# zju3dv/pvnet

Measured on NVIDIA H100. Metric: images/sec (480x640, K=9) backbone+vote, higher is better.
Workload: dtype tf32 (fp32 storage, fp32 accumulate; vote fp32/fp64)

## Files before the change

pvnet_b200/csrc/conv_col.cu:

```cuda
#include "conv_tc.cuh"
#include "ptx.cuh"

#include <cstdlib>
#include <mutex>
#include <new>

namespace pvnet {

int g_conv_mode = 0;

namespace {

constexpr int COL_TH = 16, COL_TW = 8;
constexpr int COL_THREADS = 384;
constexpr int HEAD_MAX = 64;

__host__ __device__ constexpr int head_pitch(int hc) { return hc <= 8 ? 8 : (hc <= 24 ? 24 : 40); }
constexpr int HEAD_CPITCH = COL_TH * COL_TW + 4;
__host__ __device__ constexpr int head_stage_floats(int hc)
{
    return COL_TH * COL_TW * head_pitch(hc) > hc * HEAD_CPITCH ? COL_TH * COL_TW * head_pitch(hc) : hc * HEAD_CPITCH;
}
__host__ __device__ constexpr int head_stage_bytes(int hc) { return (head_stage_floats(hc) * 4 + COL_TH * COL_TW + 127) & ~127; }

struct ColGeom {
    int Ho, Wo, tiles_x, tiles_y, total_tiles;
    int cin_chunks, cin_pad;
    int split_chunk;
    int pad_l, pad_t;
    int stages;
    int resident;
    int out_cs, out_co, res_cs, res_co;
    int act, round_out;
    int head_cout, head_seg, mask_esz;
    int head_nhwc;
};

__device__ __forceinline__ void head_store_tile(const ColGeom &g, uint32_t sv, uint32_t sm, float *head_out, void *mask,
                                                int img, int y0, int x0, int tid, int nthr)
{
    const int hc = g.head_cout, pp = head_pitch(hc);
    const int nx = min(COL_TW, g.Wo - x0), ny = min(COL_TH, g.Ho - y0);
    const size_t npix = (size_t)g.Ho * g.Wo;
    const bool vec = (reinterpret_cast<uintptr_t>(head_out) & 15) == 0 && (g.head_nhwc ? hc % 4 == 0 : g.Wo % 4 == 0);
    for (int u = tid; u < 32 * hc; u += nthr) {
        if (g.head_nhwc) {
            const int r = u / (2 * hc), e0 = 4 * (u - r * 2 * hc);
            if (r >= ny) continue;
            float *dst = head_out + (((size_t)img * g.Ho + y0 + r) * g.Wo + x0) * hc + e0;
            if (vec) {
                const int col = e0 / hc;
                if (col < nx)
                    *reinterpret_cast<float4 *>(dst) = ptx::lds128(sv + 4u * (uint32_t)((r * COL_TW + col) * pp + e0 - col * hc));
            } else {
#pragma unroll
                for (int i = 0; i < 4; ++i) {
                    const int col = (e0 + i) / hc;
                    if (col < nx) dst[i] = ptx::lds32(sv + 4u * (uint32_t)((r * COL_TW + col) * pp + e0 + i - col * hc));
                }
            }
        } else {
            const int co = u >> 5, r = (u >> 1) & 15, xo = 4 * (u & 1);
            if (r >= ny) continue;
            float *dst = head_out + ((size_t)img * hc + co) * npix + (size_t)(y0 + r) * g.Wo + x0 + xo;
            const uint32_t src = sv + 4u * (uint32_t)(co * HEAD_CPITCH + r * COL_TW + xo);
            if (vec) {
                if (xo < nx) *reinterpret_cast<float4 *>(dst) = ptx::lds128(src);
            } else {
#pragma unroll
                for (int i = 0; i < 4; ++i)
                    if (xo + i < nx) dst[i] = ptx::lds32(src + 4u * i);
            }
        }
    }
    if (!mask) return;
    for (int p = tid; p < COL_TH * COL_TW; p += nthr) {
        const int r = p / COL_TW, c = p % COL_TW;
        if (r >= ny || c >= nx) continue;
        const size_t pix = ((size_t)img * g.Ho + y0 + r) * g.Wo + x0 + c;
        const uint32_t v = ptx::lds8(sm + (uint32_t)p);
        if (g.mask_esz == 8) reinterpret_cast<long long *>(mask)[pix] = v;
        else reinterpret_cast<unsigned char *>(mask)[pix] = (unsigned char)v;
    }
}

template <int KC, bool HEAD, int KH, int BN, bool WIDE = false>
__global__ void __launch_bounds__(COL_THREADS, 1)
    k_conv_col(const __grid_constant__ CUtensorMap tmA, const __grid_constant__ CUtensorMap tmA2,
               const __grid_constant__ CUtensorMap tmB, const __grid_constant__ CUtensorMap tmBw, const __grid_constant__ ColGeom g,
               const float *__restrict__ bias, const float *__restrict__ res, float *__restrict__ out,
               const float *__restrict__ head_w, const float *__restrict__ head_b, float *__restrict__ head_out,
               void *__restrict__ mask)
{
    static_assert(!HEAD || BN == 32, "fused head: 32 input channels");
    static_assert(!HEAD || KC == 8, "fused head: convraw.0's 8-channel chunks");
    static_assert((KC == 16) == (KH == 4), "16-channel chunks are the 4x4 stem's, and only its");
    static_assert(!WIDE || (HEAD && KC == 8 && KH == 3), "wide first source: convraw.0 form only");
    constexpr int ROWB = KC * 4;
    constexpr int B_TILE = BN * ROWB;
    constexpr int PITCH = COL_TW + KH - 1;
    constexpr int A_BOX = (COL_TH + KH - 1) * PITCH * ROWB;
    constexpr int A_BYTES = (A_BOX + 1023) & ~1023;
    constexpr int WIDE_BOX = (COL_TH + KH - 1) * PITCH * 128;
    constexpr int WIDE_BYTES = (WIDE_BOX + 1023) & ~1023;
    extern __shared__ uint8_t smem_raw[];
    uint8_t *smem = reinterpret_cast<uint8_t *>((reinterpret_cast<uintptr_t>(smem_raw) + 1023) & ~uintptr_t(1023));
    const int n_btiles = KH * KH * g.cin_chunks;
    const int n_loads = WIDE ? 2 : g.cin_chunks;
    const int stage_bytes = WIDE ? WIDE_BYTES : A_BYTES + (g.resident ? 0 : KH * KH * B_TILE);
    uint8_t *sB = smem;
    uint8_t *sA = smem + (g.resident ? (size_t)n_btiles * B_TILE : 0);
    uint8_t *sH = sA + (size_t)g.stages * stage_bytes;
    uint8_t *sHS = sH + (HEAD ? 4096 : 0);
    const int hs_bytes = HEAD ? head_stage_bytes(g.head_cout) : 0;
    uint64_t *wfull = reinterpret_cast<uint64_t *>(sHS + 2 * hs_bytes);
    uint64_t *full = wfull + 1;
    uint64_t *empty = full + g.stages;
    uint64_t *hstaged = empty + g.stages;
    uint64_t *hfree = hstaged + 2;
    float *s_bias = reinterpret_cast<float *>(empty + g.stages + (HEAD ? 4 : 0));
    float *s_head = s_bias + 64;
    constexpr int STORE_THREADS = 96;

    const int warp = threadIdx.x >> 5, lane = threadIdx.x & 31;
    if (threadIdx.x == 0) {
        ptx::mbar_init(wfull, 1);
        for (int s = 0; s < g.stages; ++s) {
            ptx::mbar_init(&full[s], 1);
            ptx::mbar_init(&empty[s], 8);
        }
        if (HEAD)
            for (int b = 0; b < 2; ++b) {
                ptx::mbar_init(&hstaged[b], 256);
                ptx::mbar_init(&hfree[b], STORE_THREADS);
            }
        ptx::fence_barrier_init();
    }
    for (int i = threadIdx.x; i < BN; i += blockDim.x) s_bias[i] = bias[i];
    if (HEAD) {
        for (int i = threadIdx.x; i < 32; i += blockDim.x) s_head[i] = i < g.head_cout ? head_b[i] : 0.f;
        for (int i = threadIdx.x; i < 32 * 32; i += blockDim.x) {
            const int n = i >> 5, p = i & 31, q = p & 7;
            const int k = (p & ~7) + (q < 4 ? 2 * q : 2 * (q - 4) + 1);
            const float v = n < g.head_cout ? head_w[n * 32 + k] : 0.f;
            *reinterpret_cast<float *>(sH + ptx::swizzle_off((uint32_t)(n * 128 + p * 4), 128)) = v;
        }
        ptx::fence_proxy_async();
    }
    __syncthreads();
    const int tiles_per_img = g.tiles_x * g.tiles_y;

    if (warp >= 8) {
        const int pw = warp - 8;
        if (pw == 0 && lane == 0 && g.resident) {
            ptx::mbar_arrive_expect_tx(wfull, (uint32_t)(n_btiles * B_TILE));
            for (int cc = WIDE ? g.split_chunk : 0; cc < g.cin_chunks; ++cc)
                for (int t = 0; t < KH * KH; ++t)
                    ptx::tma_load_2d(sB + (size_t)(cc * KH * KH + t) * B_TILE, &tmB, wfull, t * g.cin_pad + cc * KC, 0);
            if (WIDE)
                for (int t = 0; t < KH * KH; ++t) ptx::tma_load_2d(sB + (size_t)t * BN * 128, &tmBw, wfull, t * g.cin_pad, 0);
        }
        if (HEAD && pw != 0) {
            const int tid = threadIdx.x - 9 * 32;
            int it = 0;
            for (int tile = blockIdx.x; tile < g.total_tiles; tile += gridDim.x, ++it) {
                const int b = it & 1;
                const int img = tile / tiles_per_img;
                const int trem = tile - img * tiles_per_img;
                const int tyi = trem / g.tiles_x, txi = trem - tyi * g.tiles_x;
                const uint32_t buf = ptx::smem_u32(sHS) + (uint32_t)(b * hs_bytes);
                ptx::mbar_wait(&hstaged[b], (uint32_t)(it >> 1) & 1u);
                head_store_tile(g, buf, buf + 4u * (uint32_t)head_stage_floats(g.head_cout), head_out, mask, img, tyi * COL_TH,
                                txi * COL_TW, tid, STORE_THREADS);
                ptx::mbar_arrive(&hfree[b]);
            }
            return;
        }
        if (pw != 0) return;
        int s = 0;
        uint32_t ph = 0;
        const uint32_t tx_bytes = (uint32_t)(A_BOX + (g.resident ? 0 : KH * KH * B_TILE));
        for (int tile = blockIdx.x; tile < g.total_tiles; tile += gridDim.x) {
            const int img = tile / tiles_per_img;
            const int trem = tile - img * tiles_per_img;
            const int tyi = trem / g.tiles_x, txi = trem - tyi * g.tiles_x;
            const int y0 = tyi * COL_TH, x0 = txi * COL_TW;
            for (int cc = 0; cc < n_loads; ++cc) {
                uint8_t *st = sA + (size_t)s * stage_bytes;
                if (WIDE) {
                    if (pw == 0 && lane == 0) {
                        ptx::mbar_wait(&empty[s], ph ^ 1u);
                        ptx::mbar_arrive_expect_tx(&full[s], (uint32_t)(cc == 0 ? WIDE_BOX : A_BOX));
                        ptx::tma_load_4d(st, cc == 0 ? &tmA : &tmA2, &full[s], 0, x0 - g.pad_l, y0 - g.pad_t, img);
                    }
                    __syncwarp();
                } else if (pw == 0) {
                    if (lane == 0) {
                        ptx::mbar_wait(&empty[s], ph ^ 1u);
                        ptx::mbar_arrive_expect_tx(&full[s], tx_bytes);
                        if (cc < g.split_chunk)
                            ptx::tma_load_4d(st, &tmA, &full[s], cc * KC, x0 - g.pad_l, y0 - g.pad_t, img);
                        else
                            ptx::tma_load_4d(st, &tmA2, &full[s], (cc - g.split_chunk) * KC, x0 - g.pad_l, y0 - g.pad_t, img);
                        if (!g.resident)
                            for (int t = 0; t < KH * KH; ++t)
                                ptx::tma_load_2d(st + A_BYTES + (size_t)t * B_TILE, &tmB, &full[s], t * g.cin_pad + cc * KC, 0);
                    }
                    __syncwarp();
                }
                if (++s == g.stages) {
                    s = 0;
                    ph ^= 1u;
                }
            }
        }
        return;
    }

    const int wg = warp >> 2, wq = warp & 3;
    const int g8 = lane >> 2, t4 = lane & 3;
    const uint32_t sA_u = ptx::smem_u32(sA), sB_u = ptx::smem_u32(sB);
    if (g.resident) ptx::mbar_wait(wfull, 0);
    int s = 0;
    uint32_t ph = 0;
    int it = 0;
    for (int tile = blockIdx.x; tile < g.total_tiles; tile += gridDim.x, ++it) {
        float acc[BN / 2];
#pragma unroll
        for (int i = 0; i < BN / 2; ++i) acc[i] = 0.f;
        int prev = -1;
        for (int cc = 0; cc < n_loads; ++cc) {
            ptx::mbar_wait(&full[s], ph);
            const uint32_t a0 = sA_u + (uint32_t)s * (uint32_t)stage_bytes;
            ptx::wgmma_fence();
            if (WIDE && cc == 0) {
                const uint64_t ad0 = ptx::make_kmajor_desc(a0 + (uint32_t)(8 * wg * PITCH * 128), 128, PITCH * 128);
                const uint64_t bd0 = ptx::make_kmajor_desc(sB_u, 128);
#pragma unroll
                for (int ks = 0; ks < 4; ++ks)
#pragma unroll
                    for (int t = 0; t < KH * KH; ++t)
                        ptx::Wgmma<BN>::ss(acc, ad0 + (uint64_t)(((t / KH) * PITCH + t % KH) * 128 / 16 + 2 * ks),
                                           bd0 + (uint64_t)(t * (BN * 128) / 16 + 2 * ks), (t | ks) != 0 ? 1u : 0u);
            } else {
                const int c8 = WIDE ? g.split_chunk : cc;
                const uint32_t b0 = g.resident ? sB_u + (uint32_t)(c8 * KH * KH * B_TILE) : a0 + (uint32_t)A_BYTES;
                const uint64_t ad0 = ptx::make_kmajor_desc(a0 + (uint32_t)(8 * wg * PITCH * ROWB), ROWB, PITCH * ROWB);
                const uint64_t bd0 = ptx::make_kmajor_desc(b0, ROWB);
#pragma unroll
                for (int t = 0; t < KH * KH; ++t) {
                    const uint64_t ad = ad0 + (uint64_t)(((t / KH) * PITCH + t % KH) * ROWB / 16);
                    const uint64_t bd = bd0 + (uint64_t)(t * B_TILE / 16);
#pragma unroll
                    for (int ks = 0; ks < KC / 8; ++ks)
                        ptx::Wgmma<BN>::ss(acc, ad + (uint64_t)(2 * ks), bd + (uint64_t)(2 * ks), (c8 | t | ks) != 0 ? 1u : 0u);
                }
            }
            ptx::wgmma_commit();
            ptx::wgmma_wait<1>();
            ptx::fence_regs(acc);
            if (prev >= 0 && lane == 0) ptx::mbar_arrive(&empty[prev]);
            prev = s;
            if (++s == g.stages) {
                s = 0;
                ph ^= 1u;
            }
        }
        ptx::wgmma_wait<0>();
        ptx::fence_regs(acc);
        if (lane == 0) ptx::mbar_arrive(&empty[prev]);

        const int img = tile / tiles_per_img;
        const int trem = tile - img * tiles_per_img;
        const int tyi = trem / g.tiles_x, txi = trem - tyi * g.tiles_x;
        const int ty = 8 * wg + 2 * wq;
        if constexpr (!HEAD) {
            bool ok[2];
            size_t pix[2];
#pragma unroll
            for (int h = 0; h < 2; ++h) {
                const int y = tyi * COL_TH + ty + h, x = txi * COL_TW + g8;
                ok[h] = y < g.Ho && x < g.Wo;
                pix[h] = ok[h] ? ((size_t)img * g.Ho + y) * g.Wo + x : 0;
            }
            float2 rv[2][BN / 8];
            if (res) {
#pragma unroll
                for (int h = 0; h < 2; ++h)
#pragma unroll
                    for (int j = 0; j < BN / 8; ++j)
                        rv[h][j] = ok[h] ? __ldg(reinterpret_cast<const float2 *>(res + pix[h] * g.res_cs + g.res_co + 8 * j + 2 * t4))
                                         : make_float2(0.f, 0.f);
            }
#pragma unroll
            for (int h = 0; h < 2; ++h) {
                if (!ok[h]) continue;
                float *optr = out + pix[h] * g.out_cs + g.out_co;
#pragma unroll
                for (int j = 0; j < BN / 8; ++j) {
                    const int c = 8 * j + 2 * t4;
                    float2 v = make_float2(acc[4 * j + 2 * h] + s_bias[c], acc[4 * j + 2 * h + 1] + s_bias[c + 1]);
                    if (res) {
                        v.x += rv[h][j].x;
                        v.y += rv[h][j].y;
                    }
                    v.x = epi_act(v.x, g.act, g.round_out);
                    v.y = epi_act(v.y, g.act, g.round_out);
                    *reinterpret_cast<float2 *>(optr + c) = v;
                }
            }
        } else {
            uint32_t a2[4][4];
#pragma unroll
            for (int j = 0; j < 4; ++j)
#pragma unroll
                for (int f = 0; f < 4; ++f) {
                    const int r = 4 * j + ((f & 1) << 1) + (f >> 1);
                    const int c = 8 * j + 2 * t4 + (f >> 1);
                    a2[j][f] = __float_as_uint(ptx::round_tf32(epi_act(acc[r] + s_bias[c], g.act, g.round_out)));
                }
            float hacc[16];
#pragma unroll
            for (int i = 0; i < 16; ++i) hacc[i] = 0.f;
            const uint64_t hd = ptx::make_kmajor_desc(ptx::smem_u32(sH), 128);
            ptx::wgmma_fence();
#pragma unroll
            for (int j = 0; j < 4; ++j) ptx::Wgmma<32>::rs(hacc, a2[j], hd + (uint64_t)(2 * j), j != 0 ? 1u : 0u);
            ptx::wgmma_commit();
            ptx::wgmma_wait<0>();
            ptx::fence_regs(hacc);
            const int hc = g.head_cout, pp = head_pitch(hc);
            const uint32_t sv = ptx::smem_u32(sHS) + (uint32_t)((it & 1) * hs_bytes);
            const uint32_t sm = sv + 4u * (uint32_t)head_stage_floats(hc);
            ptx::mbar_wait(&hfree[it & 1], ((uint32_t)(it >> 1) & 1u) ^ 1u);
#pragma unroll
            for (int h = 0; h < 2; ++h) {
                const uint32_t p = (uint32_t)((ty + h) * COL_TW + g8);
                float best = -INFINITY;
                int best_c = 0;
#pragma unroll
                for (int j = 0; j < 4; ++j) {
                    const int co = 8 * j + 2 * t4;
                    float val[2];
#pragma unroll
                    for (int e = 0; e < 2; ++e) {
                        val[e] = hacc[4 * j + 2 * h + e] + s_head[co + e];
                        if (co + e < g.head_seg && val[e] > best) {
                            best = val[e];
                            best_c = co + e;
                        }
                    }
                    if (co < hc) {
                        if (g.head_nhwc) {
                            ptx::sts64(sv + 4u * (p * pp + co), make_float2(val[0], val[1]));
                        } else {
                            ptx::sts32(sv + 4u * (co * HEAD_CPITCH + p), val[0]);
                            if (co + 1 < hc) ptx::sts32(sv + 4u * ((co + 1) * HEAD_CPITCH + p), val[1]);
                        }
                    }
                }
#pragma unroll
                for (int o = 1; o < 4; o <<= 1) {
                    const float ob = __shfl_xor_sync(0xffffffffu, best, o);
                    const int oc = __shfl_xor_sync(0xffffffffu, best_c, o);
                    if (ob > best || (ob == best && oc < best_c)) {
                        best = ob;
                        best_c = oc;
                    }
                }
                if (t4 == 0) ptx::sts8(sm + p, (uint32_t)best_c);
            }
            ptx::mbar_arrive(&hstaged[it & 1]);
        }
    }
}

struct ColPlan {
    CUtensorMap tmA, tmA2, tmB, tmBw;
    ColGeom g;
    int kc, ksize, head, bn, wide;
    unsigned grid;
    size_t smem;
    const float *bias, *res;
    float *out;
    HeadDesc hd;
};

constexpr size_t SMEM_LIMIT = 227 * 1024;

int col_kc(int Cin) { return Cin % 32 == 0 ? 32 : (Cin == 16 ? 16 : 8); }
int col_cin_pad(int Cin) { return Cin == 16 ? 16 : (Cin + 31) / 32 * 32; }

size_t col_smem(int kc, int ksize, int cin_chunks, int bn, int stages, bool head, bool resident)
{
    const size_t rowb = (size_t)kc * 4;
    const size_t a_box = (size_t)(COL_TH + ksize - 1) * (COL_TW + ksize - 1) * rowb;
    const size_t a = (a_box + 1023) & ~(size_t)1023, bt = (size_t)bn * rowb;
    return 1024 + (resident ? (size_t)ksize * ksize * cin_chunks * bt : 0) +
           (size_t)stages * (a + (resident ? 0 : (size_t)ksize * ksize * bt)) + (head ? 4096 : 0) +
           (size_t)(1 + 2 * stages) * 8 + (64 + 32) * 4;
}

template <int KC, bool HEAD, int KH, int BN, bool WIDE = false>
int col_launch(const ColPlan &p, cudaStream_t s)
{
    if (p.bn != BN || p.kc != KC || p.ksize != KH || p.head != (HEAD ? 1 : 0) || p.wide != (WIDE ? 1 : 0)) {
        set_error("conv(col): no kernel instantiation for this plan (Cout %d, chunk %d, ksize %d)", p.bn, p.kc, p.ksize);
        return PVNET_E_STATE;
    }
    auto fn = k_conv_col<KC, HEAD, KH, BN, WIDE>;
    const cudaError_t attr_err = ensure_max_smem((const void *)fn, (int)SMEM_LIMIT);
    PV_CUDA(attr_err);
    const HeadDesc &h = p.hd;
    fn<<<p.grid, COL_THREADS, p.smem, s>>>(p.tmA, p.tmA2, p.tmB, p.tmBw, p.g, p.bias, p.res, p.out, p.head ? h.w : nullptr,
                                           p.head ? h.bias : nullptr, p.head ? h.out_nchw : nullptr,
                                           p.head ? h.mask : nullptr);
    PV_LAUNCHED("k_conv_col");
    return PVNET_OK;
}

}

bool conv_col_eligible(const ConvDesc &d)
{
    if ((d.ksize != 3 && d.ksize != 4) || d.stride != 1 || d.dilation != 1 || d.Cout > 64 || d.Cout % 32 != 0)
        return false;
    const int cin = d.Cin + d.Cin2;
    const int kc = col_kc(cin);
    if (d.Cin % kc != 0 || d.Cin2 % kc != 0) return false;
    if ((d.ksize == 4) != (kc == 16)) return false;
    return col_smem(kc, d.ksize, (cin + kc - 1) / kc, d.Cout, 2, true, false) <= SMEM_LIMIT;
}

size_t conv_col_plan_size() { return sizeof(ColPlan); }

int conv_col_plan_at(const ConvDesc &d, const HeadDesc *head, void *storage)
{
    ColPlan *p = new (storage) ColPlan();
    PV_CHECK_ARG(conv_col_eligible(d), "conv(col): layer not eligible for the column kernel");
    PV_CHECK_ARG(d.in && d.w && d.bias && (d.out || head), "conv(col): null pointer");
    PV_CHECK_ARG(d.in_cs % 4 == 0 && d.in_co % 4 == 0 && d.out_cs % 4 == 0 && d.out_co % 4 == 0,
                 "conv(col): channel strides/offsets must be multiples of 4 floats");
    PV_CHECK_ARG(!d.res || (d.res_cs % 4 == 0 && d.res_co % 4 == 0), "conv(col): residual stride/offset alignment");
    PV_CHECK_ARG(!head || (d.Cout == 32 && col_kc(d.Cin + d.Cin2) == 8 && head->cout >= 1 && head->cout <= 32 && head->w && head->bias &&
                           head->out_nchw && (!head->mask || head->mask_esz == 1 || head->mask_esz == 8)),
                 "conv(col): bad fused-head description");
    const int kc = col_kc(d.Cin + d.Cin2);
    ColGeom &g = p->g;
    g.pad_l = g.pad_t = d.ksize == 4 ? 2 : 1;
    g.Ho = d.H;
    g.Wo = d.W;
    g.tiles_x = (d.W + COL_TW - 1) / COL_TW;
    g.tiles_y = (d.H + COL_TH - 1) / COL_TH;
    g.total_tiles = g.tiles_x * g.tiles_y * d.b;
    g.cin_chunks = (d.Cin + d.Cin2) / kc;
    g.split_chunk = d.in2 ? d.Cin / kc : g.cin_chunks;
    g.cin_pad = col_cin_pad(d.Cin + d.Cin2);
    g.out_cs = d.out_cs;
    g.out_co = d.out_co;
    g.res_cs = d.res_cs;
    g.res_co = d.res_co;
    g.act = d.act;
    g.round_out = d.round_out;
    g.head_cout = head ? head->cout : 0;
    g.head_seg = head ? head->seg_dim : 0;
    g.mask_esz = head ? head->mask_esz : 0;
    g.head_nhwc = 0;
    const bool hd = head != nullptr;
    const size_t hs = hd ? 2 * (size_t)head_stage_bytes(head->cout) + 4 * 8 : 0;
    bool wide = hd && d.in2 && d.Cin == 32 && d.Cin2 == 8 && kc == 8 && d.ksize == 3;
    const size_t wx = col_smem(32, 3, 0, 0, 1, false, false) - col_smem(8, 3, 0, 0, 1, false, false);
    int stages = 8;
    bool resident = true;
    while (stages > 2 && col_smem(kc, d.ksize, g.cin_chunks, d.Cout, stages, hd, true) + hs + (wide ? stages * wx : 0) > SMEM_LIMIT)
        --stages;
    if (col_smem(kc, d.ksize, g.cin_chunks, d.Cout, stages, hd, true) + hs + (wide ? stages * wx : 0) > SMEM_LIMIT) {
        wide = false;
        resident = false;
        stages = 8;
        while (stages > 2 && col_smem(kc, d.ksize, g.cin_chunks, d.Cout, stages, hd, false) + hs > SMEM_LIMIT) --stages;
    }
    g.stages = stages;
    g.resident = resident ? 1 : 0;
    p->smem = col_smem(kc, d.ksize, g.cin_chunks, d.Cout, stages, hd, resident) + hs + (wide ? stages * wx : 0);
    p->wide = wide ? 1 : 0;
    PV_CHECK_ARG(p->smem <= SMEM_LIMIT, "conv(col): layer does not fit in shared memory");
    p->kc = kc;
    p->ksize = d.ksize;
    p->bn = d.Cout;
    p->head = hd ? 1 : 0;
    if (head) p->hd = *head;
    {
        const float *base = d.in + d.in_co;
        cuuint64_t dims[4] = {(cuuint64_t)d.Cin, (cuuint64_t)d.W, (cuuint64_t)d.H, (cuuint64_t)d.b};
        cuuint64_t strides[3] = {(cuuint64_t)d.in_cs * 4, (cuuint64_t)d.W * d.in_cs * 4,
                                 (cuuint64_t)d.H * d.W * d.in_cs * 4};
        const int akc = wide ? 32 : kc;
        cuuint32_t box[4] = {(cuuint32_t)akc, (cuuint32_t)(COL_TW + d.ksize - 1), (cuuint32_t)(COL_TH + d.ksize - 1), 1};
        int rc = tma_encode(&p->tmA, base, 4, dims, strides, box, akc * 4);
        if (rc) return rc;
        p->tmA2 = p->tmA;
    }
    if (d.in2) {
        PV_CHECK_ARG(d.in2_cs % 4 == 0 && d.in2_co % 4 == 0 && d.Cin2 > 0, "conv(col): second source stride/offset alignment");
        cuuint64_t dims[4] = {(cuuint64_t)d.Cin2, (cuuint64_t)d.W, (cuuint64_t)d.H, (cuuint64_t)d.b};
        cuuint64_t strides[3] = {(cuuint64_t)d.in2_cs * 4, (cuuint64_t)d.W * d.in2_cs * 4,
                                 (cuuint64_t)d.H * d.W * d.in2_cs * 4};
        cuuint32_t box[4] = {(cuuint32_t)kc, (cuuint32_t)(COL_TW + d.ksize - 1), (cuuint32_t)(COL_TH + d.ksize - 1), 1};
        int rc = tma_encode(&p->tmA2, d.in2 + d.in2_co, 4, dims, strides, box, kc * 4);
        if (rc) return rc;
    }
    {
        cuuint64_t dims[2] = {(cuuint64_t)d.ksize * d.ksize * g.cin_pad, (cuuint64_t)d.Cout};
        cuuint64_t strides[1] = {(cuuint64_t)d.ksize * d.ksize * g.cin_pad * 4};
        cuuint32_t box[2] = {(cuuint32_t)kc, (cuuint32_t)d.Cout};
        int rc = tma_encode(&p->tmB, d.w, 2, dims, strides, box, kc * 4);
        if (rc) return rc;
        p->tmBw = p->tmB;
        if (wide) {
            box[0] = 32;
            if ((rc = tma_encode(&p->tmBw, d.w, 2, dims, strides, box, 128))) return rc;
        }
    }
    PV_CHECK_ARG(!head || (uintptr_t)head->w % 16 == 0, "conv(col): head weights must be 16-byte aligned");
    long long grid = (long long)sm_count();
    if (grid > g.total_tiles) grid = g.total_tiles;
    p->grid = (unsigned)grid;
    p->bias = d.bias;
    p->res = d.res;
    p->out = d.out;
    return PVNET_OK;
}

void conv_col_set_head_ptrs(void *storage, float *out_nchw, void *mask, int mask_esz, int nhwc)
{
    ColPlan *p = static_cast<ColPlan *>(storage);
    p->g.head_nhwc = nhwc;
    p->hd.out_nchw = out_nchw;
    p->hd.mask = mask;
    p->hd.mask_esz = mask_esz;
    p->g.mask_esz = mask_esz;
}

int conv_col_launch_at(const void *storage, cudaStream_t s)
{
    const ColPlan &p = *static_cast<const ColPlan *>(storage);
    if (p.wide) return col_launch<8, true, 3, 32, true>(p, s);
    if (p.head) return col_launch<8, true, 3, 32>(p, s);
    const bool n64 = p.bn == 64;
    if (p.ksize == 4) return n64 ? col_launch<16, false, 4, 64>(p, s) : col_launch<16, false, 4, 32>(p, s);
    if (p.kc == 32) return n64 ? col_launch<32, false, 3, 64>(p, s) : col_launch<32, false, 3, 32>(p, s);
    return n64 ? col_launch<8, false, 3, 64>(p, s) : col_launch<8, false, 3, 32>(p, s);
}

}

extern "C" {
int pvnet_conv_set_mode(int mode)
{
    PV_CHECK_ARG(mode >= 0 && mode <= 2, "mode must be 0, 1 or 2");
    pvnet::g_conv_mode = mode;
    return PVNET_OK;
}
}
```

Before: 1723.

## Widen fused-head convraw.0 tiles to 16 columns and load second source as 32-wide box

For the wide convraw.0 path with the fused segmentation head, the spatial tile is widened from 8 to 16 columns. Each warpgroup now holds two accumulator halves that share every B descriptor, and the head GEMM and argmax run over both halves. The second 8-channel source is now loaded with a 32-channel box, and its weights are loaded as a second 32-wide tile. The loop issues only the first k-step for that source. The aim is fewer tiles, more weight reuse per tile and fewer pipeline iterations, at the cost of more accumulator registers, larger stage buffers and 32-wide reads of an 8-channel input.

Result: no change. 1734, median of 6 (+0.7%).

```diff
diff --git a/pvnet_b200/csrc/conv_col.cu b/pvnet_b200/csrc/conv_col.cu
--- a/pvnet_b200/csrc/conv_col.cu
+++ b/pvnet_b200/csrc/conv_col.cu
@@ -12,16 +12,20 @@
 namespace {
 
 constexpr int COL_TH = 16, COL_TW = 8;
+constexpr int WIDE_TW = 16;
 constexpr int COL_THREADS = 384;
 constexpr int HEAD_MAX = 64;
 
 __host__ __device__ constexpr int head_pitch(int hc) { return hc <= 8 ? 8 : (hc <= 24 ? 24 : 40); }
-constexpr int HEAD_CPITCH = COL_TH * COL_TW + 4;
-__host__ __device__ constexpr int head_stage_floats(int hc)
-{
-    return COL_TH * COL_TW * head_pitch(hc) > hc * HEAD_CPITCH ? COL_TH * COL_TW * head_pitch(hc) : hc * HEAD_CPITCH;
-}
-__host__ __device__ constexpr int head_stage_bytes(int hc) { return (head_stage_floats(hc) * 4 + COL_TH * COL_TW + 127) & ~127; }
+__host__ __device__ constexpr int head_cpitch(int tpix) { return tpix + 4; }
+__host__ __device__ constexpr int head_stage_floats(int hc, int tpix)
+{
+    return tpix * head_pitch(hc) > hc * head_cpitch(tpix) ? tpix * head_pitch(hc) : hc * head_cpitch(tpix);
+}
+__host__ __device__ constexpr int head_stage_bytes(int hc, int tpix)
+{
+    return (head_stage_floats(hc, tpix) * 4 + tpix + 127) & ~127;
+}
 
 struct ColGeom {
     int Ho, Wo, tiles_x, tiles_y, total_tiles;
@@ -36,34 +40,36 @@
     int head_nhwc;
 };
 
+template <int TW>
 __device__ __forceinline__ void head_store_tile(const ColGeom &g, uint32_t sv, uint32_t sm, float *head_out, void *mask,
                                                 int img, int y0, int x0, int tid, int nthr)
 {
-    const int hc = g.head_cout, pp = head_pitch(hc);
-    const int nx = min(COL_TW, g.Wo - x0), ny = min(COL_TH, g.Ho - y0);
+    constexpr int TPIX = COL_TH * TW, CPITCH = head_cpitch(TPIX);
+    const int hc = g.head_cout, pp = head_pitch(hc), row_units = TW * hc / 4;
+    const int nx = min(TW, g.Wo - x0), ny = min(COL_TH, g.Ho - y0);
     const size_t npix = (size_t)g.Ho * g.Wo;
     const bool vec = (reinterpret_cast<uintptr_t>(head_out) & 15) == 0 && (g.head_nhwc ? hc % 4 == 0 : g.Wo % 4 == 0);
-    for (int u = tid; u < 32 * hc; u += nthr) {
+    for (int u = tid; u < TPIX / 4 * hc; u += nthr) {
         if (g.head_nhwc) {
-            const int r = u / (2 * hc), e0 = 4 * (u - r * 2 * hc);
+            const int r = u / row_units, e0 = 4 * (u - r * row_units);
             if (r >= ny) continue;
             float *dst = head_out + (((size_t)img * g.Ho + y0 + r) * g.Wo + x0) * hc + e0;
             if (vec) {
                 const int col = e0 / hc;
                 if (col < nx)
-                    *reinterpret_cast<float4 *>(dst) = ptx::lds128(sv + 4u * (uint32_t)((r * COL_TW + col) * pp + e0 - col * hc));
+                    *reinterpret_cast<float4 *>(dst) = ptx::lds128(sv + 4u * (uint32_t)((r * TW + col) * pp + e0 - col * hc));
             } else {
 #pragma unroll
                 for (int i = 0; i < 4; ++i) {
                     const int col = (e0 + i) / hc;
-                    if (col < nx) dst[i] = ptx::lds32(sv + 4u * (uint32_t)((r * COL_TW + col) * pp + e0 + i - col * hc));
+                    if (col < nx) dst[i] = ptx::lds32(sv + 4u * (uint32_t)((r * TW + col) * pp + e0 + i - col * hc));
                 }
             }
         } else {
-            const int co = u >> 5, r = (u >> 1) & 15, xo = 4 * (u & 1);
+            const int co = u / (TPIX / 4), r = (u / (TW / 4)) % COL_TH, xo = 4 * (u % (TW / 4));
             if (r >= ny) continue;
             float *dst = head_out + ((size_t)img * hc + co) * npix + (size_t)(y0 + r) * g.Wo + x0 + xo;
-            const uint32_t src = sv + 4u * (uint32_t)(co * HEAD_CPITCH + r * COL_TW + xo);
+            const uint32_t src = sv + 4u * (uint32_t)(co * CPITCH + r * TW + xo);
             if (vec) {
                 if (xo < nx) *reinterpret_cast<float4 *>(dst) = ptx::lds128(src);
             } else {
@@ -74,8 +80,8 @@
         }
     }
     if (!mask) return;
-    for (int p = tid; p < COL_TH * COL_TW; p += nthr) {
-        const int r = p / COL_TW, c = p % COL_TW;
+    for (int p = tid; p < TPIX; p += nthr) {
+        const int r = p / TW, c = p % TW;
         if (r >= ny || c >= nx) continue;
         const size_t pix = ((size_t)img * g.Ho + y0 + r) * g.Wo + x0 + c;
         const uint32_t v = ptx::lds8(sm + (uint32_t)p);
@@ -96,23 +102,26 @@
     static_assert(!HEAD || KC == 8, "fused head: convraw.0's 8-channel chunks");
     static_assert((KC == 16) == (KH == 4), "16-channel chunks are the 4x4 stem's, and only its");
     static_assert(!WIDE || (HEAD && KC == 8 && KH == 3), "wide first source: convraw.0 form only");
+    constexpr int TW = WIDE ? WIDE_TW : COL_TW;
+    constexpr int NH = TW / 8;
     constexpr int ROWB = KC * 4;
     constexpr int B_TILE = BN * ROWB;
-    constexpr int PITCH = COL_TW + KH - 1;
+    constexpr int PITCH = TW + KH - 1;
     constexpr int A_BOX = (COL_TH + KH - 1) * PITCH * ROWB;
     constexpr int A_BYTES = (A_BOX + 1023) & ~1023;
     constexpr int WIDE_BOX = (COL_TH + KH - 1) * PITCH * 128;
     constexpr int WIDE_BYTES = (WIDE_BOX + 1023) & ~1023;
+    constexpr int W_TILE = BN * 128;
     extern __shared__ uint8_t smem_raw[];
     uint8_t *smem = reinterpret_cast<uint8_t *>((reinterpret_cast<uintptr_t>(smem_raw) + 1023) & ~uintptr_t(1023));
-    const int n_btiles = KH * KH * g.cin_chunks;
+    const int w_bytes = WIDE ? 2 * KH * KH * W_TILE : KH * KH * g.cin_chunks * B_TILE;
     const int n_loads = WIDE ? 2 : g.cin_chunks;
     const int stage_bytes = WIDE ? WIDE_BYTES : A_BYTES + (g.resident ? 0 : KH * KH * B_TILE);
     uint8_t *sB = smem;
-    uint8_t *sA = smem + (g.resident ? (size_t)n_btiles * B_TILE : 0);
+    uint8_t *sA = smem + (g.resident ? (size_t)w_bytes : 0);
     uint8_t *sH = sA + (size_t)g.stages * stage_bytes;
     uint8_t *sHS = sH + (HEAD ? 4096 : 0);
-    const int hs_bytes = HEAD ? head_stage_bytes(g.head_cout) : 0;
+    const int hs_bytes = HEAD ? head_stage_bytes(g.head_cout, COL_TH * TW) : 0;
     uint64_t *wfull = reinterpret_cast<uint64_t *>(sHS + 2 * hs_bytes);
     uint64_t *full = wfull + 1;
     uint64_t *empty = full + g.stages;
@@ -153,12 +162,17 @@
     if (warp >= 8) {
         const int pw = warp - 8;
         if (pw == 0 && lane == 0 && g.resident) {
-            ptx::mbar_arrive_expect_tx(wfull, (uint32_t)(n_btiles * B_TILE));
-            for (int cc = WIDE ? g.split_chunk : 0; cc < g.cin_chunks; ++cc)
-                for (int t = 0; t < KH * KH; ++t)
-                    ptx::tma_load_2d(sB + (size_t)(cc * KH * KH + t) * B_TILE, &tmB, wfull, t * g.cin_pad + cc * KC, 0);
-            if (WIDE)
-                for (int t = 0; t < KH * KH; ++t) ptx::tma_load_2d(sB + (size_t)t * BN * 128, &tmBw, wfull, t * g.cin_pad, 0);
+            ptx::mbar_arrive_expect_tx(wfull, (uint32_t)w_bytes);
+            if (WIDE) {
+                for (int t = 0; t < KH * KH; ++t) {
+                    ptx::tma_load_2d(sB + (size_t)t * W_TILE, &tmBw, wfull, t * g.cin_pad, 0);
+                    ptx::tma_load_2d(sB + (size_t)(KH * KH + t) * W_TILE, &tmBw, wfull, t * g.cin_pad + 32, 0);
+                }
+            } else {
+                for (int cc = 0; cc < g.cin_chunks; ++cc)
+                    for (int t = 0; t < KH * KH; ++t)
+                        ptx::tma_load_2d(sB + (size_t)(cc * KH * KH + t) * B_TILE, &tmB, wfull, t * g.cin_pad + cc * KC, 0);
+            }
         }
         if (HEAD && pw != 0) {
             const int tid = threadIdx.x - 9 * 32;
@@ -170,8 +184,8 @@
                 const int tyi = trem / g.tiles_x, txi = trem - tyi * g.tiles_x;
                 const uint32_t buf = ptx::smem_u32(sHS) + (uint32_t)(b * hs_bytes);
                 ptx::mbar_wait(&hstaged[b], (uint32_t)(it >> 1) & 1u);
-                head_store_tile(g, buf, buf + 4u * (uint32_t)head_stage_floats(g.head_cout), head_out, mask, img, tyi * COL_TH,
-                                txi * COL_TW, tid, STORE_THREADS);
+                head_store_tile<TW>(g, buf, buf + 4u * (uint32_t)head_stage_floats(g.head_cout, COL_TH * TW), head_out, mask,
+                                    img, tyi * COL_TH, txi * TW, tid, STORE_THREADS);
                 ptx::mbar_arrive(&hfree[b]);
             }
             return;
@@ -184,13 +198,13 @@
             const int img = tile / tiles_per_img;
             const int trem = tile - img * tiles_per_img;
             const int tyi = trem / g.tiles_x, txi = trem - tyi * g.tiles_x;
-            const int y0 = tyi * COL_TH, x0 = txi * COL_TW;
+            const int y0 = tyi * COL_TH, x0 = txi * TW;
             for (int cc = 0; cc < n_loads; ++cc) {
                 uint8_t *st = sA + (size_t)s * stage_bytes;
                 if (WIDE) {
                     if (pw == 0 && lane == 0) {
                         ptx::mbar_wait(&empty[s], ph ^ 1u);
-                        ptx::mbar_arrive_expect_tx(&full[s], (uint32_t)(cc == 0 ? WIDE_BOX : A_BOX));
+                        ptx::mbar_arrive_expect_tx(&full[s], (uint32_t)WIDE_BOX);
                         ptx::tma_load_4d(st, cc == 0 ? &tmA : &tmA2, &full[s], 0, x0 - g.pad_l, y0 - g.pad_t, img);
                     }
                     __syncwarp();
@@ -225,26 +239,34 @@
     uint32_t ph = 0;
     int it = 0;
     for (int tile = blockIdx.x; tile < g.total_tiles; tile += gridDim.x, ++it) {
-        float acc[BN / 2];
-#pragma unroll
-        for (int i = 0; i < BN / 2; ++i) acc[i] = 0.f;
+        float acc[NH][BN / 2];
+#pragma unroll
+        for (int h = 0; h < NH; ++h)
+#pragma unroll
+            for (int i = 0; i < BN / 2; ++i) acc[h][i] = 0.f;
         int prev = -1;
         for (int cc = 0; cc < n_loads; ++cc) {
             ptx::mbar_wait(&full[s], ph);
             const uint32_t a0 = sA_u + (uint32_t)s * (uint32_t)stage_bytes;
             ptx::wgmma_fence();
-            if (WIDE && cc == 0) {
+            if constexpr (WIDE) {
                 const uint64_t ad0 = ptx::make_kmajor_desc(a0 + (uint32_t)(8 * wg * PITCH * 128), 128, PITCH * 128);
-                const uint64_t bd0 = ptx::make_kmajor_desc(sB_u, 128);
-#pragma unroll
-                for (int ks = 0; ks < 4; ++ks)
-#pragma unroll
-                    for (int t = 0; t < KH * KH; ++t)
-                        ptx::Wgmma<BN>::ss(acc, ad0 + (uint64_t)(((t / KH) * PITCH + t % KH) * 128 / 16 + 2 * ks),
-                                           bd0 + (uint64_t)(t * (BN * 128) / 16 + 2 * ks), (t | ks) != 0 ? 1u : 0u);
+                const uint64_t bd0 = ptx::make_kmajor_desc(sB_u + (uint32_t)(cc * KH * KH * W_TILE), 128);
+#pragma unroll
+                for (int ks = 0; ks < 4; ++ks) {
+                    if (cc != 0 && ks != 0) break;
+#pragma unroll
+                    for (int t = 0; t < KH * KH; ++t) {
+                        const uint64_t ad = ad0 + (uint64_t)(((t / KH) * PITCH + t % KH) * 128 / 16 + 2 * ks);
+                        const uint64_t bd = bd0 + (uint64_t)(t * W_TILE / 16 + 2 * ks);
+                        const uint32_t accumulate = (cc | t | ks) != 0 ? 1u : 0u;
+#pragma unroll
+                        for (int h = 0; h < NH; ++h)
+                            ptx::Wgmma<BN>::ss(acc[h], ad + (uint64_t)(h * 8 * 128 / 16), bd, accumulate);
+                    }
+                }
             } else {
-                const int c8 = WIDE ? g.split_chunk : cc;
-                const uint32_t b0 = g.resident ? sB_u + (uint32_t)(c8 * KH * KH * B_TILE) : a0 + (uint32_t)A_BYTES;
+                const uint32_t b0 = g.resident ? sB_u + (uint32_t)(cc * KH * KH * B_TILE) : a0 + (uint32_t)A_BYTES;
                 const uint64_t ad0 = ptx::make_kmajor_desc(a0 + (uint32_t)(8 * wg * PITCH * ROWB), ROWB, PITCH * ROWB);
                 const uint64_t bd0 = ptx::make_kmajor_desc(b0, ROWB);
 #pragma unroll
@@ -253,12 +275,13 @@
                     const uint64_t bd = bd0 + (uint64_t)(t * B_TILE / 16);
 #pragma unroll
                     for (int ks = 0; ks < KC / 8; ++ks)
-                        ptx::Wgmma<BN>::ss(acc, ad + (uint64_t)(2 * ks), bd + (uint64_t)(2 * ks), (c8 | t | ks) != 0 ? 1u : 0u);
+                        ptx::Wgmma<BN>::ss(acc[0], ad + (uint64_t)(2 * ks), bd + (uint64_t)(2 * ks), (cc | t | ks) != 0 ? 1u : 0u);
                 }
             }
             ptx::wgmma_commit();
             ptx::wgmma_wait<1>();
-            ptx::fence_regs(acc);
+#pragma unroll
+            for (int h = 0; h < NH; ++h) ptx::fence_regs(acc[h]);
             if (prev >= 0 && lane == 0) ptx::mbar_arrive(&empty[prev]);
             prev = s;
             if (++s == g.stages) {
@@ -267,7 +290,8 @@
             }
         }
         ptx::wgmma_wait<0>();
-        ptx::fence_regs(acc);
+#pragma unroll
+        for (int h = 0; h < NH; ++h) ptx::fence_regs(acc[h]);
         if (lane == 0) ptx::mbar_arrive(&empty[prev]);
 
         const int img = tile / tiles_per_img;
@@ -279,7 +303,7 @@
             size_t pix[2];
 #pragma unroll
             for (int h = 0; h < 2; ++h) {
-                const int y = tyi * COL_TH + ty + h, x = txi * COL_TW + g8;
+                const int y = tyi * COL_TH + ty + h, x = txi * TW + g8;
                 ok[h] = y < g.Ho && x < g.Wo;
                 pix[h] = ok[h] ? ((size_t)img * g.Ho + y) * g.Wo + x : 0;
             }
@@ -299,7 +323,7 @@
 #pragma unroll
                 for (int j = 0; j < BN / 8; ++j) {
                     const int c = 8 * j + 2 * t4;
-                    float2 v = make_float2(acc[4 * j + 2 * h] + s_bias[c], acc[4 * j + 2 * h + 1] + s_bias[c + 1]);
+                    float2 v = make_float2(acc[0][4 * j + 2 * h] + s_bias[c], acc[0][4 * j + 2 * h + 1] + s_bias[c + 1]);
                     if (res) {
                         v.x += rv[h][j].x;
                         v.y += rv[h][j].y;
@@ -310,65 +334,86 @@
                 }
             }
         } else {
-            uint32_t a2[4][4];
-#pragma unroll
-            for (int j = 0; j < 4; ++j)
-#pragma unroll
-                for (int f = 0; f < 4; ++f) {
-                    const int r = 4 * j + ((f & 1) << 1) + (f >> 1);
-                    const int c = 8 * j + 2 * t4 + (f >> 1);
-                    a2[j][f] = __float_as_uint(ptx::round_tf32(epi_act(acc[r] + s_bias[c], g.act, g.round_out)));
-                }
-            float hacc[16];
-#pragma unroll
-            for (int i = 0; i < 16; ++i) hacc[i] = 0.f;
+            uint32_t a2[NH][4][4];
+#pragma unroll
+            for (int hf = 0; hf < NH; ++hf)
+#pragma unroll
+                for (int j = 0; j < 4; ++j)
+#pragma unroll
+                    for (int f = 0; f < 4; ++f) {
+                        const int r = 4 * j + ((f & 1) << 1) + (f >> 1);
+                        const int c = 8 * j + 2 * t4 + (f >> 1);
+                        a2[hf][j][f] = __float_as_uint(ptx::round_tf32(epi_act(acc[hf][r] + s_bias[c], g.act, g.round_out)));
+                    }
+            float hacc[NH][16];
+#pragma unroll
+            for (int hf = 0; hf < NH; ++hf)
+#pragma unroll
+                for (int i = 0; i < 16; ++i) hacc[hf][i] = 0.f;
             const uint64_t hd = ptx::make_kmajor_desc(ptx::smem_u32(sH), 128);
             ptx::wgmma_fence();
 #pragma unroll
-            for (int j = 0; j < 4; ++j) ptx::Wgmma<32>::rs(hacc, a2[j], hd + (uint64_t)(2 * j), j != 0 ? 1u : 0u);
+            for (int hf = 0; hf < NH; ++hf)
+#pragma unroll
+                for (int j = 0; j < 4; ++j) ptx::Wgmma<32>::rs(hacc[hf], a2[hf][j], hd + (uint64_t)(2 * j), j != 0 ? 1u : 0u);
             ptx::wgmma_commit();
             ptx::wgmma_wait<0>();
-            ptx::fence_regs(hacc);
+#pragma unroll
+            for (int hf = 0; hf < NH; ++hf) ptx::fence_regs(hacc[hf]);
+            constexpr int CPITCH = head_cpitch(COL_TH * TW);
             const int hc = g.head_cout, pp = head_pitch(hc);
             const uint32_t sv = ptx::smem_u32(sHS) + (uint32_t)((it & 1) * hs_bytes);
-            const uint32_t sm = sv + 4u * (uint32_t)head_stage_floats(hc);
+            const uint32_t sm = sv + 4u * (uint32_t)head_stage_floats(hc, COL_TH * TW);
+            float best[2 * NH];
+            int best_c[2 * NH];
+#pragma unroll
+            for (int q = 0; q < 2 * NH; ++q) {
+                const int hf = q >> 1, h = q & 1;
+                best[q] = -INFINITY;
+                best_c[q] = 0;
+#pragma unroll
+                for (int j = 0; j < 4; ++j)
+#pragma unroll
+                    for (int e = 0; e < 2; ++e) {
+                        const int co = 8 * j + 2 * t4 + e;
+                        float &v = hacc[hf][4 * j + 2 * h + e];
+                        v += s_head[co];
+                        if (co < g.head_seg && v > best[q]) {
+                            best[q] = v;
+                            best_c[q] = co;
+                        }
+                    }
+            }
+#pragma unroll
+            for (int o = 1; o < 4; o <<= 1)
+#pragma unroll
+                for (int q = 0; q < 2 * NH; ++q) {
+                    const float ob = __shfl_xor_sync(0xffffffffu, best[q], o);
+                    const int oc = __shfl_xor_sync(0xffffffffu, best_c[q], o);
+                    if (ob > best[q] || (ob == best[q] && oc < best_c[q])) {
+                        best[q] = ob;
+                        best_c[q] = oc;
+                    }
+                }
             ptx::mbar_wait(&hfree[it & 1], ((uint32_t)(it >> 1) & 1u) ^ 1u);
 #pragma unroll
-            for (int h = 0; h < 2; ++h) {
-                const uint32_t p = (uint32_t)((ty + h) * COL_TW + g8);
-                float best = -INFINITY;
-                int best_c = 0;
+            for (int q = 0; q < 2 * NH; ++q) {
+                const int hf = q >> 1, h = q & 1;
+                const uint32_t p = (uint32_t)((ty + h) * TW + 8 * hf + g8);
 #pragma unroll
                 for (int j = 0; j < 4; ++j) {
                     const int co = 8 * j + 2 * t4;
-                    float val[2];
-#pragma unroll
-                    for (int e = 0; e < 2; ++e) {
-                        val[e] = hacc[4 * j + 2 * h + e] + s_head[co + e];
-                        if (co + e < g.head_seg && val[e] > best) {
-                            best = val[e];
-                            best_c = co + e;
-                        }
-                    }
+                    const float v0 = hacc[hf][4 * j + 2 * h], v1 = hacc[hf][4 * j + 2 * h + 1];
                     if (co < hc) {
                         if (g.head_nhwc) {
-                            ptx::sts64(sv + 4u * (p * pp + co), make_float2(val[0], val[1]));
+                            ptx::sts64(sv + 4u * (p * pp + co), make_float2(v0, v1));
                         } else {
-                            ptx::sts32(sv + 4u * (co * HEAD_CPITCH + p), val[0]);
-                            if (co + 1 < hc) ptx::sts32(sv + 4u * ((co + 1) * HEAD_CPITCH + p), val[1]);
+                            ptx::sts32(sv + 4u * (co * CPITCH + p), v0);
+                            if (co + 1 < hc) ptx::sts32(sv + 4u * ((co + 1) * CPITCH + p), v1);
                         }
                     }
                 }
-#pragma unroll
-                for (int o = 1; o < 4; o <<= 1) {
-                    const float ob = __shfl_xor_sync(0xffffffffu, best, o);
-                    const int oc = __shfl_xor_sync(0xffffffffu, best_c, o);
-                    if (ob > best || (ob == best && oc < best_c)) {
-                        best = ob;
-                        best_c = oc;
-                    }
-                }
-                if (t4 == 0) ptx::sts8(sm + p, (uint32_t)best_c);
+                if (t4 == 0) ptx::sts8(sm + p, (uint32_t)best_c[q]);
             }
             ptx::mbar_arrive(&hstaged[it & 1]);
         }
@@ -391,10 +436,10 @@
 int col_kc(int Cin) { return Cin % 32 == 0 ? 32 : (Cin == 16 ? 16 : 8); }
 int col_cin_pad(int Cin) { return Cin == 16 ? 16 : (Cin + 31) / 32 * 32; }
 
-size_t col_smem(int kc, int ksize, int cin_chunks, int bn, int stages, bool head, bool resident)
+size_t col_smem(int kc, int ksize, int cin_chunks, int bn, int stages, bool head, bool resident, int tw = COL_TW)
 {
     const size_t rowb = (size_t)kc * 4;
-    const size_t a_box = (size_t)(COL_TH + ksize - 1) * (COL_TW + ksize - 1) * rowb;
+    const size_t a_box = (size_t)(COL_TH + ksize - 1) * (tw + ksize - 1) * rowb;
     const size_t a = (a_box + 1023) & ~(size_t)1023, bt = (size_t)bn * rowb;
     return 1024 + (resident ? (size_t)ksize * ksize * cin_chunks * bt : 0) +
            (size_t)stages * (a + (resident ? 0 : (size_t)ksize * ksize * bt)) + (head ? 4096 : 0) +
@@ -450,9 +495,6 @@
     g.pad_l = g.pad_t = d.ksize == 4 ? 2 : 1;
     g.Ho = d.H;
     g.Wo = d.W;
-    g.tiles_x = (d.W + COL_TW - 1) / COL_TW;
-    g.tiles_y = (d.H + COL_TH - 1) / COL_TH;
-    g.total_tiles = g.tiles_x * g.tiles_y * d.b;
     g.cin_chunks = (d.Cin + d.Cin2) / kc;
     g.split_chunk = d.in2 ? d.Cin / kc : g.cin_chunks;
     g.cin_pad = col_cin_pad(d.Cin + d.Cin2);
@@ -467,23 +509,30 @@
     g.mask_esz = head ? head->mask_esz : 0;
     g.head_nhwc = 0;
     const bool hd = head != nullptr;
-    const size_t hs = hd ? 2 * (size_t)head_stage_bytes(head->cout) + 4 * 8 : 0;
     bool wide = hd && d.in2 && d.Cin == 32 && d.Cin2 == 8 && kc == 8 && d.ksize == 3;
-    const size_t wx = col_smem(32, 3, 0, 0, 1, false, false) - col_smem(8, 3, 0, 0, 1, false, false);
+    auto smem_for = [&](bool w, int stages, bool resident) {
+        const int tw = w ? WIDE_TW : COL_TW;
+        const size_t hs = hd ? 2 * (size_t)head_stage_bytes(head->cout, COL_TH * tw) + 4 * 8 : 0;
+        return (w ? col_smem(32, 3, 2, d.Cout, stages, true, true, tw)
+                  : col_smem(kc, d.ksize, g.cin_chunks, d.Cout, stages, hd, resident, tw)) + hs;
+    };
     int stages = 8;
     bool resident = true;
-    while (stages > 2 && col_smem(kc, d.ksize, g.cin_chunks, d.Cout, stages, hd, true) + hs + (wide ? stages * wx : 0) > SMEM_LIMIT)
-        --stages;
-    if (col_smem(kc, d.ksize, g.cin_chunks, d.Cout, stages, hd, true) + hs + (wide ? stages * wx : 0) > SMEM_LIMIT) {
+    while (stages > 2 && smem_for(wide, stages, true) > SMEM_LIMIT) --stages;
+    if (smem_for(wide, stages, true) > SMEM_LIMIT) {
         wide = false;
         resident = false;
         stages = 8;
-        while (stages > 2 && col_smem(kc, d.ksize, g.cin_chunks, d.Cout, stages, hd, false) + hs > SMEM_LIMIT) --stages;
+        while (stages > 2 && smem_for(false, stages, false) > SMEM_LIMIT) --stages;
     }
     g.stages = stages;
     g.resident = resident ? 1 : 0;
-    p->smem = col_smem(kc, d.ksize, g.cin_chunks, d.Cout, stages, hd, resident) + hs + (wide ? stages * wx : 0);
+    p->smem = smem_for(wide, stages, resident);
     p->wide = wide ? 1 : 0;
+    const int tw = wide ? WIDE_TW : COL_TW;
+    g.tiles_x = (d.W + tw - 1) / tw;
+    g.tiles_y = (d.H + COL_TH - 1) / COL_TH;
+    g.total_tiles = g.tiles_x * g.tiles_y * d.b;
     PV_CHECK_ARG(p->smem <= SMEM_LIMIT, "conv(col): layer does not fit in shared memory");
     p->kc = kc;
     p->ksize = d.ksize;
@@ -496,7 +545,7 @@
         cuuint64_t strides[3] = {(cuuint64_t)d.in_cs * 4, (cuuint64_t)d.W * d.in_cs * 4,
                                  (cuuint64_t)d.H * d.W * d.in_cs * 4};
         const int akc = wide ? 32 : kc;
-        cuuint32_t box[4] = {(cuuint32_t)akc, (cuuint32_t)(COL_TW + d.ksize - 1), (cuuint32_t)(COL_TH + d.ksize - 1), 1};
+        cuuint32_t box[4] = {(cuuint32_t)akc, (cuuint32_t)(tw + d.ksize - 1), (cuuint32_t)(COL_TH + d.ksize - 1), 1};
         int rc = tma_encode(&p->tmA, base, 4, dims, strides, box, akc * 4);
         if (rc) return rc;
         p->tmA2 = p->tmA;
@@ -506,8 +555,9 @@
         cuuint64_t dims[4] = {(cuuint64_t)d.Cin2, (cuuint64_t)d.W, (cuuint64_t)d.H, (cuuint64_t)d.b};
         cuuint64_t strides[3] = {(cuuint64_t)d.in2_cs * 4, (cuuint64_t)d.W * d.in2_cs * 4,
                                  (cuuint64_t)d.H * d.W * d.in2_cs * 4};
-        cuuint32_t box[4] = {(cuuint32_t)kc, (cuuint32_t)(COL_TW + d.ksize - 1), (cuuint32_t)(COL_TH + d.ksize - 1), 1};
-        int rc = tma_encode(&p->tmA2, d.in2 + d.in2_co, 4, dims, strides, box, kc * 4);
+        const int akc = wide ? 32 : kc;
+        cuuint32_t box[4] = {(cuuint32_t)akc, (cuuint32_t)(tw + d.ksize - 1), (cuuint32_t)(COL_TH + d.ksize - 1), 1};
+        int rc = tma_encode(&p->tmA2, d.in2 + d.in2_co, 4, dims, strides, box, akc * 4);
         if (rc) return rc;
     }
     {
```
